# MrTornado24/FENeRF

Measured on NVIDIA H100. Metric: rendered faces/sec at 128px x 24 samples/ray, higher is better.
Workload: dtype f16 operands / f32 accumulate (wgmma) + f32 refinement

## Files before the change

### fenerf_b200/csrc/mapping.cu

```cuda
#include "common.cuh"

namespace fn {

namespace {

constexpr int kMaxB = 32;
constexpr unsigned kFull = 0xffffffffu;

struct HiddenArgs {
    const float* w[4];
    const float* b[4];
    const float* z;
    float* h_out;
    int B, z_dim;
};

constexpr int kChunkB = 8;

__global__ void __launch_bounds__(256) mapping_hidden_kernel(HiddenArgs a) {
    extern __shared__ __align__(16) float xs[];
    const int warp = threadIdx.x >> 5, lane = threadIdx.x & 31;
    const int B = a.B;
    float* x0 = xs;
    float* x1 = xs + (size_t)B * 512;
    for (int i = threadIdx.x; i < B * a.z_dim; i += blockDim.x) x0[(i / a.z_dim) * 512 + (i % a.z_dim)] = a.z[i];
    __syncthreads();
    int K = a.z_dim;
    for (int layer = 0; layer < 4; ++layer) {
        const float* W = a.w[layer];
        const float* bias = a.b[layer];
        const float* xin = (layer & 1) ? x1 : x0;
        float* xout = (layer & 1) ? x0 : x1;
#pragma unroll 1
        for (int og = 0; og < 4; ++og) {
        float4 wreg[8][4];
#pragma unroll
        for (int o = 0; o < 8; ++o)
#pragma unroll
            for (int it = 0; it < 4; ++it) {
                const int k = lane * 4 + it * 128;
                wreg[o][it] = k < K ? __ldg(reinterpret_cast<const float4*>(W + (size_t)(warp * 32 + og * 8 + o) * K + k)) : make_float4(0.f, 0.f, 0.f, 0.f);
            }
#pragma unroll
        for (int o = 0; o < 8; ++o) {
            const int f = warp * 32 + og * 8 + o;
            for (int b0 = 0; b0 < B; b0 += kChunkB) {
                float acc[kChunkB];
#pragma unroll
                for (int b = 0; b < kChunkB; ++b) acc[b] = 0.f;
#pragma unroll
                for (int it = 0; it < 4; ++it) {
                    const int k = lane * 4 + it * 128;
                    if (k < K) {
                        const float4 wv = wreg[o][it];
#pragma unroll
                        for (int b = 0; b < kChunkB; ++b)
                            if (b0 + b < B) {
                                const float4 xv = *reinterpret_cast<const float4*>(xin + (b0 + b) * 512 + k);
                                acc[b] = fmaf(wv.x, xv.x, fmaf(wv.y, xv.y, fmaf(wv.z, xv.z, fmaf(wv.w, xv.w, acc[b]))));
                            }
                    }
                }
#pragma unroll
                for (int b = 0; b < kChunkB; ++b)
                    if (b0 + b < B) {
                        float v = acc[b];
#pragma unroll
                        for (int off = 16; off > 0; off >>= 1) v += __shfl_xor_sync(kFull, v, off);
                        v += bias[f];
                        v = v > 0.f ? v : 0.2f * v;
                        if (lane == 0) {
                            if (layer == 3) a.h_out[(b0 + b) * 256 + f] = v;
                            else xout[(b0 + b) * 512 + f] = v;
                        }
                    }
            }
        }
        }
        __syncthreads();
        K = 256;
    }
}

struct OutArgs {
    const float* w;
    const float* b;
    const float* h;
    const float* avg_f;
    const float* avg_p;
    float* film;
    int B, n_layers, layer0, n_film_total;
    float psi;
};

__global__ void __launch_bounds__(256) mapping_out_kernel(OutArgs a) {
    extern __shared__ __align__(16) float hs[];
    const int B = a.B;
    for (int i = threadIdx.x; i < B * 256; i += blockDim.x) hs[i] = a.h[i];
    __syncthreads();
    const int warp = threadIdx.x >> 5, lane = threadIdx.x & 31;
    const int half = a.n_layers * 256, n_out = 2 * half;
    for (int r = blockIdx.x * 8 + warp; r < n_out; r += gridDim.x * 8) {
        const float4 w0 = *reinterpret_cast<const float4*>(a.w + (size_t)r * 256 + lane * 8);
        const float4 w1 = *reinterpret_cast<const float4*>(a.w + (size_t)r * 256 + lane * 8 + 4);
        const float bias = a.b[r];
        const bool is_freq = r < half;
        const int j = is_freq ? r : r - half, l = j >> 8, f = j & 255;
        for (int b = 0; b < B; ++b) {
            const float4 x0 = *reinterpret_cast<const float4*>(hs + b * 256 + lane * 8);
            const float4 x1 = *reinterpret_cast<const float4*>(hs + b * 256 + lane * 8 + 4);
            float v = fmaf(w0.x, x0.x, fmaf(w0.y, x0.y, fmaf(w0.z, x0.z, w0.w * x0.w)));
            v = fmaf(w1.x, x1.x, fmaf(w1.y, x1.y, fmaf(w1.z, x1.z, fmaf(w1.w, x1.w, v))));
#pragma unroll
            for (int off = 16; off > 0; off >>= 1) v += __shfl_xor_sync(kFull, v, off);
            if (lane == 0) {
                v += bias;
                if (a.avg_f) {
                    const float avg = is_freq ? a.avg_f[j] : a.avg_p[j];
                    v = __fadd_rn(avg, __fmul_rn(a.psi, __fsub_rn(v, avg)));
                }
                if (is_freq) v = __fadd_rn(__fmul_rn(v, 15.f), 30.f);
                a.film[(((size_t)b * a.n_film_total + a.layer0 + l) * 2 + (is_freq ? 0 : 1)) * 256 + f] = v;
            }
        }
    }
}

}

int mapping_film(const float* const* w, const float* const* b, const float* z, int B, int z_dim, int n_layers, int layer0,
                 int n_film_total, const float* avg_f, const float* avg_p, float psi, float* h_scratch, float* film,
                 cudaStream_t st) {
    FN_REQUIRE(z_dim >= 4 && z_dim <= 512 && z_dim % 4 == 0, "z_dim %d unsupported (multiple of 4, <= 512)", z_dim);
    for (int b0 = 0; b0 < B; b0 += kMaxB) {
        const int nb = (B - b0) < kMaxB ? (B - b0) : kMaxB;
        HiddenArgs ha;
        for (int i = 0; i < 4; ++i) { ha.w[i] = w[i]; ha.b[i] = b[i]; }
        ha.z = z + (size_t)b0 * z_dim; ha.h_out = h_scratch; ha.B = nb; ha.z_dim = z_dim;
        const size_t smem_h = (size_t)2 * nb * 512 * sizeof(float);
        static std::atomic<int> set_h[kMaxDevices];
        if (smem_h > 48 * 1024) FN_CUDA_OK(ensure_dynamic_smem(mapping_hidden_kernel, set_h, (int)smem_h));
        mapping_hidden_kernel<<<1, 256, smem_h, st>>>(ha);
        FN_LAUNCH_OK("mapping_hidden_kernel");
        OutArgs oa;
        oa.w = w[4]; oa.b = b[4]; oa.h = h_scratch; oa.avg_f = avg_f; oa.avg_p = avg_p;
        oa.film = film + (size_t)b0 * n_film_total * 512; oa.B = nb; oa.n_layers = n_layers; oa.layer0 = layer0;
        oa.n_film_total = n_film_total; oa.psi = psi;
        const int rows = n_layers * 512;
        int blocks = (rows + 7) / 8;
        if (blocks > num_sms() * 2) blocks = num_sms() * 2;
        mapping_out_kernel<<<blocks, 256, (size_t)nb * 256 * sizeof(float), st>>>(oa);
        FN_LAUNCH_OK("mapping_out_kernel");
    }
    return 0;
}

}
```

### fenerf_b200/csrc/siren_fast.cu

```cuda
#include "siren_fast.cuh"

namespace fn {

int siren_fast_label_launch(const void* args, int blocks, cudaStream_t st);
int siren_fast_hd_launch(const void* args, int blocks, bool label_film, cudaStream_t st);
int siren_fast_grid_launch(const void* args, int blocks, cudaStream_t st);
int siren_fast_bridge_launch(const void* args, int blocks, cudaStream_t st);
int siren_fast_debug_launch(const void* args, int blocks, bool label_film, bool feature_head, int variant, cudaStream_t st);

namespace {

std::atomic<int> g_variant{0};
unsigned long long* g_trace = nullptr;
int g_trace_ctas = 0;

bool build_loads(const FnLayout& L, FastArgs& A, bool sigma_only) {
    A.n_loads = 0;
    auto push = [&](size_t src, uint32_t bytes) {
        if (A.n_loads < MAX_LOADS) A.loads[A.n_loads] = Load{(uint32_t)src, bytes};
        ++A.n_loads;
    };
    push(L.first_img, 2 * CHUNK);
    if (L.grid_trunk) push(L.first_img_lo, 2 * CHUNK);
    for (int l = 0; l < L.n_hidden; ++l) {
        if (l == L.trunk_hidden) {
            push(L.head_img, 4 * HEAD_CHUNK);
            if (sigma_only) return A.n_loads <= MAX_LOADS;
        }
        if (L.bridge && l == L.color0) {
            push(L.color0_ximg, 2 * CHUNK);
            continue;
        }
        push(L.hid_img[l], 2 * CHUNK);
        push(L.hid_img[l] + 2 * CHUNK, 2 * CHUNK);
        if (l == L.label_layer) push(L.label.img, (uint32_t)FN_HEAD_IMG_BYTES(L.label.img_rows));
        if (l == L.color0) push(L.color0_ximg, 2 * CHUNK);
        push(L.hid_img[l] + 4 * CHUNK, 2 * CHUNK);
        push(L.hid_img[l] + 6 * CHUNK, 2 * CHUNK);
    }
    push(L.rgb.img, (uint32_t)FN_HEAD_IMG_BYTES(L.rgb.img_rows));
    return A.n_loads <= MAX_LOADS;
}

}

int siren_fast_debug_variant(int variant, unsigned long long* trace, int trace_ctas) {
    FN_REQUIRE(variant >= 0 && variant <= 3, "unknown point-network variant %d", variant);
    FN_REQUIRE(variant < 2 || (trace && trace_ctas >= 1), "a timeline variant needs its trace buffer");
    g_trace = trace;
    g_trace_ctas = trace_ctas;
    g_variant.store(variant);
    return 0;
}

int siren_points_fast(const FnLayout& L, const unsigned char* packed, const float* points, const float* dirs, const float* film,
                      int batch, long long ppb, int dir_group, int lock_dirs, float* out, int sigma_only, cudaStream_t st,
                      float* sigma_out) {
    static_assert(sizeof(FastArgs) <= 4000, "kernel parameter block too large");
    static_assert(SMEM_TOTAL <= 232448, "one CTA per SM: 227 KB of shared memory");
    static_assert(FN_HEAD_IMG_BYTES(FN_FEAT) == SLOT_BYTES, "a feature-head image is one ring slot");
    const bool trunk_only = L.feature_head && sigma_only;
    const bool feature_head = L.feature_head && !trunk_only, label_film = L.label_film && !trunk_only;
    FN_REQUIRE(L.trunk_hidden >= 1 && L.n_hidden - L.color0 >= 1, "field needs >= 2 trunk and >= 1 colour layers");
    FN_REQUIRE(L.sigma_row < 32, "the fast path packs labels and sigma into one 32-column head (label_dim <= 31)");
    FN_REQUIRE(L.rgb.img < 0xFFFFFFFFull && L.label.img < 0xFFFFFFFFull && L.first_img_lo < 0xFFFFFFFFull,
               "packed weight images beyond 4 GB");
    FN_REQUIRE(((uintptr_t)film & 15) == 0, "the FiLM table must be 16-byte aligned");
    FastArgs a;
    memset(&a, 0, sizeof(a));
    FN_REQUIRE(build_loads(L, a, sigma_only != 0), "field too deep for the weight stream");
    a.sigma_only = sigma_only ? 1 : 0;
    a.L = L; a.packed = packed; a.points = points; a.dirs = dirs; a.film = film; a.out = out; a.sigma_out = sigma_out;
    a.ppb = ppb; a.tiles_per_batch = (ppb + TILE - 1) / TILE; a.n_tiles = a.tiles_per_batch * batch;
    a.dir_group = dir_group < 1 ? 1 : dir_group; a.lock_dirs = lock_dirs;
    if (a.n_tiles <= 0) return 0;
    FN_REQUIRE(ppb % a.dir_group == 0, "points_per_batch %lld not a multiple of dir_group %d", ppb, a.dir_group);
    const long long n_pairs = (a.n_tiles + 1) / 2;
    static std::atomic<int> attr_set[kMaxDevices];
    const int blocks = (int)(n_pairs < (long long)num_sms() ? n_pairs : (long long)num_sms());
    if (const int variant = g_variant.load()) {
        FN_REQUIRE(!L.grid_trunk && !L.bridge,
                   "the debug point-network variants do not cover fields with the grid in the trunk or a bridge");
        a.trace = g_trace;
        a.trace_ctas = g_trace_ctas;
        return siren_fast_debug_launch(&a, blocks, label_film, feature_head, variant, st);
    }
    if (L.grid_trunk) return siren_fast_grid_launch(&a, blocks, st);
    if (L.bridge) return siren_fast_bridge_launch(&a, blocks, st);
    if (feature_head) return siren_fast_hd_launch(&a, blocks, label_film, st);
    if (label_film) return siren_fast_label_launch(&a, blocks, st);
    FN_CUDA_OK(ensure_dynamic_smem(siren_fast_kernel<false>, attr_set, (int)SMEM_TOTAL));
    siren_fast_kernel<false><<<blocks, NTHREADS, SMEM_TOTAL, st>>>(a);
    FN_LAUNCH_OK("siren_fast_kernel");
    return 0;
}

}
```

### fenerf_b200/csrc/siren_fast.cuh

```cuda
#pragma once
#include "common.cuh"
#include "siren_common.cuh"
#include "sm90.cuh"

namespace fn {

namespace {

using namespace sm90;

constexpr int TILE = 64;
constexpr int NTHREADS = 384;
constexpr int PROD_WARP = 8;
constexpr int RING = 6;
constexpr uint32_t SLOT_BYTES = 32768;
constexpr int XSTRIDE = 72;
constexpr uint32_t SMEM_X = RING * SLOT_BYTES;
constexpr int FRING = 2;
constexpr uint32_t FILM_BYTES = 2 * FN_H * 4;
constexpr uint32_t SMEM_FILM = SMEM_X + 2 * TILE * XSTRIDE * 2;
constexpr uint32_t SMEM_BAR = SMEM_FILM + 2 * FRING * FILM_BYTES;
constexpr uint32_t SMEM_TOTAL = SMEM_BAR + 16 * RING + 16 + 16 * 2 * FRING;
constexpr uint32_t SMEM_XLO = SMEM_TOTAL;
constexpr int XLO_STRIDE = 32;
constexpr uint32_t SMEM_TOTAL_GRID = SMEM_XLO + 2 * TILE * XLO_STRIDE * 2;
constexpr int MAX_LOADS = 72;
constexpr uint32_t CHUNK = 16384;
constexpr uint32_t HEAD_CHUNK = 32 * 128;
constexpr uint32_t RGB_CHUNK = 8 * 128;
constexpr uint32_t FEAT_CHUNK = FN_FEAT * 128;
#ifndef FENERF_SOFT_SIN_EVERY
#define FENERF_SOFT_SIN_EVERY 0
#endif
constexpr int kSoftSinEvery = FENERF_SOFT_SIN_EVERY;
constexpr int kSoftSinSplit = 4;
constexpr int TRACE_CAP = 1024;
constexpr int TRACE_WARPS = 11;
enum TraceEvent {
    TR_PAIR = 1, TR_TURN_WAIT, TR_TURN_DONE, TR_ACQ_WAIT, TR_ACQ_DONE, TR_COMMIT, TR_MMA_DONE, TR_EPI_DONE,
    TR_FILM_WAIT, TR_FILM_DONE, TR_EMPTY_WAIT, TR_EMPTY_DONE,
};
enum TraceGroup { TG_FIRST = 0, TG_HIDDEN, TG_COLOR0, TG_TRUNK_HEAD, TG_LABEL_LAYER, TG_LABEL_HEAD, TG_OUT_HEAD };

__device__ __forceinline__ float soft_sinf(float a) {
    const float k = fmaf(a, 0.159154943f, 12582912.f);
    const float n = k - 12582912.f;
    float r = fmaf(-n, 6.28318548f, a);
    r = fmaf(-n, -1.74845553e-7f, r);
    const float r2 = r * r;
    float p = -2.041572245e-08f;
    p = fmaf(p, r2, 2.701100129e-06f);
    p = fmaf(p, r2, -1.980991656e-04f);
    p = fmaf(p, r2, 8.332454599e-03f);
    p = fmaf(p, r2, -1.666656137e-01f);
    p = fmaf(p, r2, 9.999996424e-01f);
    return r * p;
}

struct Load {
    uint32_t src;
    uint32_t bytes;
};

struct FastArgs {
    Load loads[MAX_LOADS];
    int n_loads;
    FnLayout L;
    const unsigned char* packed;
    const float* points;
    const float* dirs;
    const float* film;
    float* out;
    float* sigma_out;
    long long ppb, tiles_per_batch, n_tiles;
    int dir_group, lock_dirs;
    int sigma_only;
    unsigned long long* trace;
    int trace_ctas;
};

__device__ __forceinline__ void wg_bar(int wg) { asm volatile("bar.sync %0, 128;" ::"r"(1 + wg) : "memory"); }

template <bool kLabelFilm, bool kFeatureHead = false, int kSoftSin = kSoftSinEvery, bool kTrace = false,
          bool kGridTrunk = false, bool kBridge = false>
__global__ void __launch_bounds__(NTHREADS, 1) siren_fast_kernel(const __grid_constant__ FastArgs a) {
    extern __shared__ __align__(1024) unsigned char smem[];
    const uint32_t sbase = smem_u32(smem);
    const int warp = threadIdx.x >> 5, lane = threadIdx.x & 31;
    const uint32_t bar_full = sbase + SMEM_BAR, bar_empty = bar_full + 8 * RING, bar_turn = bar_empty + 8 * RING;
    const uint32_t bar_ffull = bar_turn + 16, bar_fempty = bar_ffull + 8 * 2 * FRING;
    unsigned long long* tbuf = nullptr;
    uint32_t tn = 0;
    if constexpr (kTrace)
        if (lane == 0 && (int)blockIdx.x < a.trace_ctas) tbuf = a.trace + ((size_t)blockIdx.x * TRACE_WARPS + warp) * TRACE_CAP;
    auto trace = [&](int kind, int group = 0) {
        if constexpr (kTrace)
            if (tbuf && tn < TRACE_CAP)
                tbuf[tn++] = ((unsigned long long)kind << 56) | ((unsigned long long)group << 48) |
                             ((unsigned long long)clock64() & ((1ull << 48) - 1));
    };
    if (threadIdx.x == 0) {
        for (int i = 0; i < RING; ++i) {
            mbar_init(bar_full + 8 * i, 1);
            mbar_init(bar_empty + 8 * i, 8);
        }
        for (int g = 0; g < 2; ++g) mbar_init(bar_turn + 8 * g, 4);
        for (int e = 0; e < 2 * FRING; ++e) {
            mbar_init(bar_ffull + 8 * e, 32);
            mbar_init(bar_fempty + 8 * e, 4);
        }
        fence_barrier_init();
    }
    __syncthreads();
    const long long n_pairs = (a.n_tiles + 1) / 2;

    if (warp >= PROD_WARP) {
        asm volatile("setmaxnreg.dec.sync.aligned.u32 40;\n" ::: "memory");
        if (warp == PROD_WARP && lane == 0) {
            uint32_t it = 0;
            for (long long pair = blockIdx.x; pair < n_pairs; pair += gridDim.x)
                for (int i = 0; i < a.n_loads; ++i, ++it) {
                    const uint32_t slot = it % RING;
                    trace(TR_EMPTY_WAIT);
                    mbar_wait(bar_empty + 8 * slot, ((it / RING) & 1u) ^ 1u);
                    trace(TR_EMPTY_DONE);
                    mbar_arrive_expect_tx(bar_full + 8 * slot, a.loads[i].bytes);
                    bulk_g2s(sbase + slot * SLOT_BYTES, a.packed + a.loads[i].src, a.loads[i].bytes, bar_full + 8 * slot);
                }
        } else if (warp == PROD_WARP + 1 || warp == PROD_WARP + 2) {
            const int g = warp - PROD_WARP - 1;
            const int n_film = 1 + (a.sigma_only ? a.L.trunk_hidden : a.L.n_hidden);
            uint32_t it = 0;
            for (long long pair = blockIdx.x; pair < n_pairs; pair += gridDim.x) {
                const long long tile = pair * 2 + g;
                const long long b = tile < a.n_tiles ? tile / a.tiles_per_batch : 0;
                const float* film_b = a.film + (size_t)b * a.L.n_film * 2 * FN_H;
                for (int i = 0; i < n_film; ++i, ++it) {
                    const uint32_t e = g * FRING + it % FRING;
                    const float2* row = reinterpret_cast<const float2*>(film_b + (size_t)i * 2 * FN_H);
                    const float2* bias = reinterpret_cast<const float2*>(a.packed + (i == 0 ? a.L.first_b : a.L.hid_b[i - 1]));
                    float4* dst = reinterpret_cast<float4*>(smem + SMEM_FILM + e * FILM_BYTES);
                    trace(TR_EMPTY_WAIT);
                    mbar_wait(bar_fempty + 8 * e, ((it / FRING) & 1u) ^ 1u);
                    trace(TR_EMPTY_DONE);
#pragma unroll 1
                    for (int k = 0; k < FN_H / 64; ++k) {
                        const int cp = lane + 32 * k;
                        const float2 f = __ldg(row + cp), p = __ldg(row + FN_H / 2 + cp), bb = __ldg(bias + cp);
                        dst[cp] = make_float4(f.x, f.y, fmaf(f.x, bb.x, p.x), fmaf(f.y, bb.y, p.y));
                    }
                    mbar_arrive(bar_ffull + 8 * e);
                }
            }
        }
        return;
    }

    asm volatile("setmaxnreg.inc.sync.aligned.u32 232;\n" ::: "memory");
    const int wg = warp >> 2, q = lane & 3;
    const int tid = threadIdx.x & 127;
    const int r0 = (warp & 3) * 16 + (lane >> 2);
    const FnLayout& L = a.L;
    const int C = L.out_dim;
    const float* sigma_w = reinterpret_cast<const float*>(a.packed + L.sigma_w);
    const float* label_w = reinterpret_cast<const float*>(a.packed + L.label_w);
    const int trunk_labels = (kLabelFilm || kFeatureHead) ? 0 : L.trunk_labels;
    const int sigma_row = kFeatureHead ? FN_FEAT_SIGMA_ROW : L.sigma_row;
    const int rgb_rows = kFeatureHead ? FN_FEAT : L.rgb.w_rows;
    const int label_rows = kFeatureHead ? FN_FEAT : L.label.w_rows;
    __half* xs = reinterpret_cast<__half*>(smem + SMEM_X) + wg * TILE * XSTRIDE;
    uint32_t it = 0;
    auto acquire = [&](uint32_t& slot) -> uint32_t {
        slot = it % RING;
        trace(TR_ACQ_WAIT);
        mbar_wait(bar_full + 8 * slot, (it / RING) & 1u);
        trace(TR_ACQ_DONE);
        ++it;
        return sbase + slot * SLOT_BYTES;
    };
    auto release = [&](uint32_t slot) {
        __syncwarp();
        if (lane == 0) mbar_arrive(bar_empty + 8 * slot);
    };
    uint32_t turns = 0;
    uint32_t fit = 0;
    auto film_acquire = [&]() -> const float4* {
        const uint32_t e = wg * FRING + fit % FRING;
        trace(TR_FILM_WAIT);
        mbar_wait(bar_ffull + 8 * e, (fit / FRING) & 1u);
        trace(TR_FILM_DONE);
        return reinterpret_cast<const float4*>(smem + SMEM_FILM + e * FILM_BYTES);
    };
    auto film_release = [&]() {
        const uint32_t e = wg * FRING + fit % FRING;
        ++fit;
        __syncwarp();
        if (lane == 0) mbar_arrive(bar_fempty + 8 * e);
    };
    auto turn_begin = [&]() {
        trace(TR_TURN_WAIT);
        mbar_wait(bar_turn + 8 * wg, (turns & 1u) ^ (wg == 0 ? 1u : 0u));
        trace(TR_TURN_DONE);
    };
    auto turn_end = [&](int group) {
        trace(TR_COMMIT, group);
        ++turns;
        __syncwarp();
        if (lane == 0) mbar_arrive(bar_turn + 8 * (wg ^ 1));
    };
    auto xfrag = [&](int s, uint32_t (&f)[4]) {
        const __half* p = xs + r0 * XSTRIDE + 16 * s + 2 * q;
        f[0] = *reinterpret_cast<const uint32_t*>(p);
        f[1] = *reinterpret_cast<const uint32_t*>(p + 8 * XSTRIDE);
        f[2] = *reinterpret_cast<const uint32_t*>(p + 8);
        f[3] = *reinterpret_cast<const uint32_t*>(p + 8 * XSTRIDE + 8);
    };

    for (long long pair = blockIdx.x; pair < n_pairs; pair += gridDim.x) {
        const long long tile = pair * 2 + wg;
        const bool tile_ok = tile < a.n_tiles;
        const long long b = tile_ok ? tile / a.tiles_per_batch : 0;
        const long long p0 = tile_ok ? (tile % a.tiles_per_batch) * TILE : a.ppb;
        trace(TR_PAIR);

        wg_bar(wg);
        if (tid < TILE) {
            float pos[3] = {0.f, 0.f, 0.f}, dir[3] = {0.f, 0.f, 0.f};
            const long long pp = p0 + tid;
            const bool valid = pp < a.ppb;
            if (valid) {
                const long long ff = b * a.ppb + pp;
#pragma unroll
                for (int i = 0; i < 3; ++i) pos[i] = __fmul_rn(a.points[ff * 3 + i], L.input_scale);
                if (a.lock_dirs) dir[2] = -1.f;
                else {
                    const long long di = b * (a.ppb / a.dir_group) + pp / a.dir_group;
#pragma unroll
                    for (int i = 0; i < 3; ++i) dir[i] = a.dirs[di * 3 + i];
                }
            }
            __align__(16) __half slots[64];
#pragma unroll
            for (int i = 0; i < 64; ++i) slots[i] = __float2half_rn(0.f);
#pragma unroll
            for (int i = 0; i < 3; ++i) {
                __half hi, lo;
                split_f16(pos[i], hi, lo);
                slots[FN_SLOT_POS + i] = hi; slots[FN_SLOT_POS + 3 + i] = lo; slots[FN_SLOT_POS + 6 + i] = hi;
                split_f16(dir[i], hi, lo);
                slots[FN_SLOT_DIR + i] = hi; slots[FN_SLOT_DIR + 3 + i] = lo; slots[FN_SLOT_DIR + 6 + i] = hi;
            }
            if constexpr (kGridTrunk) {
                __align__(16) __half lo[32];
#pragma unroll
                for (int i = 0; i < 32; ++i) lo[i] = __float2half_rn(0.f);
                if (valid) {
                    float feat[32];
                    grid_features32(reinterpret_cast<const float*>(a.packed + L.grid), L.grid_res, pos[0], pos[1], pos[2], feat);
#pragma unroll
                    for (int i = 0; i < 32; ++i) split_f16(feat[i], slots[FN_SLOT_FEAT + i], lo[i]);
                }
                __half* xlo = reinterpret_cast<__half*>(smem + SMEM_XLO) + (wg * TILE + tid) * XLO_STRIDE;
#pragma unroll
                for (int i = 0; i < 4; ++i) reinterpret_cast<uint4*>(xlo)[i] = reinterpret_cast<const uint4*>(lo)[i];
            } else if (L.grid_channels > 0 && valid && !a.sigma_only) {
                float feat[32];
                grid_features32_h(reinterpret_cast<const __half*>(a.packed + L.grid16), L.grid_res, pos[0], pos[1], pos[2], feat);
#pragma unroll
                for (int i = 0; i < 32; ++i) slots[FN_SLOT_FEAT + i] = __float2half_rn(feat[i]);
            }
#pragma unroll
            for (int i = 0; i < 8; ++i)
                reinterpret_cast<uint4*>(xs + tid * XSTRIDE)[i] = reinterpret_cast<const uint4*>(slots)[i];
        }
        wg_bar(wg);

        uint32_t act[16][4];
        uint32_t nxt[8][4];
        float d[64];
        auto film_epi = [&](const float4* fs, int h, uint32_t (&dst)[8][4]) {
#pragma unroll
            for (int j = 0; j < 16; ++j) {
                const float4 e = fs[64 * h + 4 * j + q];
                const bool soft = kSoftSin > 0 && j % (kSoftSin > 0 ? kSoftSin : 1) == kSoftSin - 1;
                auto sn = [soft](float x) { return soft ? soft_sinf(x) : __sinf(x); };
                dst[j >> 1][(j & 1) * 2] = pack_half2(sn(fmaf(e.x, d[4 * j], e.z)), sn(fmaf(e.y, d[4 * j + 1], e.w)));
                dst[j >> 1][(j & 1) * 2 + 1] = pack_half2(sn(fmaf(e.x, d[4 * j + 2], e.z)), sn(fmaf(e.y, d[4 * j + 3], e.w)));
            }
            trace(TR_EPI_DONE);
        };
        auto act_hi = [&]() -> uint32_t (&)[8][4] { return *reinterpret_cast<uint32_t (*)[8][4]>(&act[8]); };

        {
            uint32_t xf[4], slot, slot_lo = 0, w_lo = 0;
            uint32_t xg[2][4], xl[2][4];
            const float4* fs = nullptr;
            xfrag(0, xf);
            if constexpr (kGridTrunk) {
                const __half* xlo = reinterpret_cast<const __half*>(smem + SMEM_XLO) + wg * TILE * XLO_STRIDE;
#pragma unroll
                for (int s = 0; s < 2; ++s) {
                    xfrag(2 + s, xg[s]);
                    const __half* p = xlo + r0 * XLO_STRIDE + 16 * s + 2 * q;
                    xl[s][0] = *reinterpret_cast<const uint32_t*>(p);
                    xl[s][1] = *reinterpret_cast<const uint32_t*>(p + 8 * XLO_STRIDE);
                    xl[s][2] = *reinterpret_cast<const uint32_t*>(p + 8);
                    xl[s][3] = *reinterpret_cast<const uint32_t*>(p + 8 * XLO_STRIDE + 8);
                }
            }
            const uint32_t w = acquire(slot);
            if constexpr (kGridTrunk) w_lo = acquire(slot_lo);
#pragma unroll
            for (int h = 0; h < 2; ++h) {
                turn_begin();
                wg_fence();
                mma_rs_n128(d, xf, desc_kmajor(w + h * CHUNK), 0u);
                if constexpr (kGridTrunk)
#pragma unroll
                    for (int s = 0; s < 2; ++s) {
                        mma_rs_n128(d, xg[s], desc_kmajor(w + h * CHUNK + 32 * (2 + s)), 1u);
                        mma_rs_n128(d, xl[s], desc_kmajor(w + h * CHUNK + 32 * (2 + s)), 1u);
                        mma_rs_n128(d, xg[s], desc_kmajor(w_lo + h * CHUNK + 32 * (2 + s)), 1u);
                    }
                wg_commit();
                turn_end(TG_FIRST);
                wg_wait<0>();
                trace(TR_MMA_DONE);
                fence_regs(d);
                fence_regs(xf);
                if constexpr (kGridTrunk) { fence_regs(xg); fence_regs(xl); }
                if (h == 0) fs = film_acquire();
                if (h == 0) film_epi(fs, 0, nxt);
                else film_epi(fs, 1, act_hi());
            }
            release(slot);
            if constexpr (kGridTrunk) release(slot_lo);
            film_release();
#pragma unroll
            for (int s = 0; s < 8; ++s)
#pragma unroll
                for (int i = 0; i < 4; ++i) act[s][i] = nxt[s][i];
        }

        bool stop = false;
        for (int l = 0; l < L.n_hidden && !stop; ++l) {
            if (l == L.trunk_hidden) {
                float dh[16];
                uint32_t slot;
                const uint32_t w = acquire(slot);
                turn_begin();
                wg_fence();
#pragma unroll
                for (int c = 0; c < 4; ++c)
#pragma unroll
                    for (int k = 0; k < 4; ++k) mma_rs_n32(dh, act[4 * c + k], desc_kmajor(w + c * HEAD_CHUNK + 32 * k), (c | k) ? 1u : 0u);
                wg_commit();
                turn_end(TG_TRUNK_HEAD);
                wg_wait<0>();
                trace(TR_MMA_DONE);
                fence_regs(dh);
                fence_regs(act);
                release(slot);
                const float* lb = label_w + FENERF_MAX_LABEL * FN_H;
#pragma unroll
                for (int rr = 0; rr < 2; ++rr) {
                    const long long pnt = p0 + r0 + 8 * rr;
                    if (pnt >= a.ppb) continue;
                    const long long flat = b * a.ppb + pnt;
#pragma unroll
                    for (int i = 0; i < 4; ++i)
#pragma unroll
                        for (int e = 0; e < 2; ++e) {
                            const int o = 8 * i + 2 * q + e;
                            const float v = dh[4 * i + 2 * rr + e];
                            if (o < trunk_labels) {
                                if (!a.sigma_only) a.out[flat * C + o] = fmaf(v, __ldg(lb + FENERF_MAX_LABEL), __ldg(lb + o));
                            } else if (o == sigma_row && !(kBridge && L.bridge_res)) {
                                const float sig = v + __ldg(sigma_w + FN_H);
                                a.out[flat * C + (C - 1)] = sig;
                                if (a.sigma_out) a.sigma_out[flat] = sig;
                            }
                        }
                }
                if constexpr (kBridge) {
                    const float* bw = reinterpret_cast<const float*>(a.packed + L.bridge_w);
#pragma unroll
                    for (int rr = 0; rr < 2; ++rr) {
                        const float o0 = dh[2 * rr], o1 = dh[2 * rr + 1];
                        const float p2 = __shfl_xor_sync(0xffffffffu, o0, 1), p3 = __shfl_xor_sync(0xffffffffu, o1, 1);
                        if (q != 0) continue;
                        const long long pnt = p0 + r0 + 8 * rr;
                        float v[3] = {o1 + __ldg(bw + 3 * FN_H), p2 + __ldg(bw + 3 * FN_H + 1), p3 + __ldg(bw + 3 * FN_H + 2)};
                        if (L.bridge_res) {
                            if (pnt < a.ppb) {
                                const long long flat = b * a.ppb + pnt;
#pragma unroll
                                for (int j = 0; j < 3; ++j) v[j] += __fmul_rn(a.points[flat * 3 + j], L.input_scale);
                                float sig = __ldg(bw + 3 * FN_H + 6);
#pragma unroll
                                for (int j = 0; j < 3; ++j) sig = fmaf(__ldg(bw + 3 * FN_H + 3 + j), v[j], sig);
                                a.out[flat * C + (C - 1)] = sig;
                                if (a.sigma_out) a.sigma_out[flat] = sig;
                            }
                        }
                        if (!a.sigma_only) {
                            __half* row = xs + (r0 + 8 * rr) * XSTRIDE + FN_SLOT_FEAT;
#pragma unroll
                            for (int j = 0; j < 3; ++j) {
                                __half hi, lo;
                                split_f16(v[j], hi, lo);
                                row[j] = hi; row[3 + j] = lo; row[6 + j] = hi;
                            }
                        }
                    }
                    if (!a.sigma_only) wg_bar(wg);
                }
                if (a.sigma_only) { stop = true; break; }
                if constexpr (kLabelFilm) {
                    constexpr int kLabN = kFeatureHead ? FN_FEAT : 32;
                    constexpr uint32_t kLabChunk = kFeatureHead ? FEAT_CHUNK : HEAD_CHUNK;
                    float dl[kLabN / 2];
                    uint32_t slot_h = 0, w_h = 0;
                    const float4* fs = nullptr;
#pragma unroll
                    for (int h = 0; h < 2; ++h) {
                        uint32_t sl[2];
                        turn_begin();
                        wg_fence();
#pragma unroll
                        for (int sb = 0; sb < 2; ++sb) {
                            const uint32_t w = acquire(sl[sb]);
#pragma unroll
                            for (int c = 0; c < 2; ++c)
#pragma unroll
                                for (int k = 0; k < 4; ++k)
                                    mma_rs_n128(d, act[8 * sb + 4 * c + k], desc_kmajor(w + c * CHUNK + 32 * k), (sb | c | k) ? 1u : 0u);
                        }
                        wg_commit();
                        turn_end(TG_LABEL_LAYER);
                        wg_wait<0>();
                        trace(TR_MMA_DONE);
                        fence_regs(d);
                        fence_regs(act);
                        release(sl[0]);
                        release(sl[1]);
                        if (h == 0) fs = film_acquire();
                        film_epi(fs, h, nxt);
                        if (h == 0) w_h = acquire(slot_h);
                        turn_begin();
                        wg_fence();
#pragma unroll
                        for (int s = 0; s < 8; ++s) {
                            const int g = 8 * h + s;
                            const uint64_t desc = desc_kmajor(w_h + (g >> 2) * kLabChunk + 32 * (g & 3));
                            if constexpr (kFeatureHead) mma_rs_n64(dl, nxt[s], desc, (h | s) ? 1u : 0u);
                            else mma_rs_n32(dl, nxt[s], desc, (h | s) ? 1u : 0u);
                        }
                        wg_commit();
                        turn_end(TG_LABEL_HEAD);
                        wg_wait<0>();
                        trace(TR_MMA_DONE);
                        fence_regs(dl);
                        fence_regs(nxt);
                    }
                    release(slot_h);
                    film_release();
#pragma unroll
                    for (int rr = 0; rr < 2; ++rr) {
                        const long long pnt = p0 + r0 + 8 * rr;
                        if (pnt >= a.ppb) continue;
                        const long long flat = b * a.ppb + pnt;
                        const float* lbias = reinterpret_cast<const float*>(a.packed + L.label.w) + label_rows * FN_H;
#pragma unroll
                        for (int i = 0; i < kLabN / 8; ++i)
#pragma unroll
                            for (int e = 0; e < 2; ++e) {
                                const int o = 8 * i + 2 * q + e;
                                if (o < L.label.n_out) a.out[flat * C + o] = dl[4 * i + 2 * rr + e] + __ldg(lbias + o);
                            }
                    }
                    continue;
                }
            }
            const bool c0 = (l == L.color0);
            const bool narrow = kBridge && c0;
            const int nx = kBridge ? 2 : !kGridTrunk && L.grid_channels > 0 ? 3 : 1;
            uint32_t xf[3][4];
            if (c0)
#pragma unroll
                for (int s = 0; s < 3; ++s) xfrag(1 + s, xf[s]);
            uint32_t slot_x = 0, w_x = 0;
            const float4* fs = nullptr;
#pragma unroll
            for (int h = 0; h < 2; ++h) {
                uint32_t sl[2] = {0u, 0u};
                if (narrow && h == 0) w_x = acquire(slot_x);
                turn_begin();
                wg_fence();
                if (!narrow)
#pragma unroll
                    for (int sb = 0; sb < 2; ++sb) {
                        const uint32_t w = acquire(sl[sb]);
#pragma unroll
                        for (int c = 0; c < 2; ++c)
#pragma unroll
                            for (int k = 0; k < 4; ++k)
                                mma_rs_n128(d, act[8 * sb + 4 * c + k], desc_kmajor(w + c * CHUNK + 32 * k), (sb | c | k) ? 1u : 0u);
                    }
                if (c0) {
                    if (h == 0 && !narrow) w_x = acquire(slot_x);
#pragma unroll
                    for (int s = 0; s < 3; ++s)
                        if (s < nx) mma_rs_n128(d, xf[s], desc_kmajor(w_x + h * CHUNK + 32 * (1 + s)), (narrow && s == 0) ? 0u : 1u);
                }
                wg_commit();
                turn_end(c0 ? TG_COLOR0 : TG_HIDDEN);
                wg_wait<0>();
                trace(TR_MMA_DONE);
                fence_regs(d);
                fence_regs(act);
                fence_regs(xf);
                if (!narrow) {
                    release(sl[0]);
                    release(sl[1]);
                }
                if (c0 && h == 1) release(slot_x);
                if (h == 0) fs = film_acquire();
                if (h == 0) film_epi(fs, 0, nxt);
                else film_epi(fs, 1, act_hi());
            }
            film_release();
#pragma unroll
            for (int s = 0; s < 8; ++s)
#pragma unroll
                for (int i = 0; i < 4; ++i) act[s][i] = nxt[s][i];
        }
        if (stop) continue;

        if constexpr (kFeatureHead) {
            float dr[32];
            uint32_t slot;
            const uint32_t w = acquire(slot);
            turn_begin();
            wg_fence();
#pragma unroll
            for (int c = 0; c < 4; ++c)
#pragma unroll
                for (int k = 0; k < 4; ++k) mma_rs_n64(dr, act[4 * c + k], desc_kmajor(w + c * FEAT_CHUNK + 32 * k), (c | k) ? 1u : 0u);
            wg_commit();
            turn_end(TG_OUT_HEAD);
            wg_wait<0>();
            trace(TR_MMA_DONE);
            fence_regs(dr);
            fence_regs(act);
            release(slot);
            const float* rgb_b = reinterpret_cast<const float*>(a.packed + L.rgb.w) + rgb_rows * FN_H;
#pragma unroll
            for (int rr = 0; rr < 2; ++rr) {
                const long long pnt = p0 + r0 + 8 * rr;
                if (pnt >= a.ppb) continue;
                const long long flat = b * a.ppb + pnt;
#pragma unroll
                for (int i = 0; i < 8; ++i)
#pragma unroll
                    for (int e = 0; e < 2; ++e) {
                        const int o = 8 * i + 2 * q + e;
                        a.out[flat * C + L.label_dim + o] = dr[4 * i + 2 * rr + e] + __ldg(rgb_b + o);
                    }
            }
            continue;
        }
        {
            float dr[4];
            uint32_t slot;
            const uint32_t w = acquire(slot);
            turn_begin();
            wg_fence();
#pragma unroll
            for (int c = 0; c < 4; ++c)
#pragma unroll
                for (int k = 0; k < 4; ++k) mma_rs_n8(dr, act[4 * c + k], desc_kmajor(w + c * RGB_CHUNK + 32 * k), (c | k) ? 1u : 0u);
            wg_commit();
            turn_end(TG_OUT_HEAD);
            wg_wait<0>();
            trace(TR_MMA_DONE);
            fence_regs(dr);
            fence_regs(act);
            release(slot);
            const float* rgb_b = reinterpret_cast<const float*>(a.packed + L.rgb.w) + rgb_rows * FN_H;
#pragma unroll
            for (int rr = 0; rr < 2; ++rr) {
                const long long pnt = p0 + r0 + 8 * rr;
                if (pnt >= a.ppb) continue;
                const long long flat = b * a.ppb + pnt;
#pragma unroll
                for (int e = 0; e < 2; ++e) {
                    const int o = 2 * q + e;
                    if (o < 3) {
                        const float x = dr[2 * rr + e] + __ldg(rgb_b + o);
                        a.out[flat * C + L.label_dim + o] = __fdividef(1.f, 1.f + __expf(-x));
                    }
                }
            }
        }
    }
}

}

}
```

### fenerf_b200/csrc/siren_fast_debug.cu

```cuda
#include "siren_fast.cuh"

namespace fn {

namespace {

template <bool kLabelFilm, bool kFeatureHead, int kSoftSin, bool kTrace>
int launch(const FastArgs& a, int blocks, cudaStream_t st) {
    static std::atomic<int> attr_set[kMaxDevices];
    FN_CUDA_OK(ensure_dynamic_smem(siren_fast_kernel<kLabelFilm, kFeatureHead, kSoftSin, kTrace>, attr_set, (int)SMEM_TOTAL));
    siren_fast_kernel<kLabelFilm, kFeatureHead, kSoftSin, kTrace><<<blocks, NTHREADS, SMEM_TOTAL, st>>>(a);
    FN_LAUNCH_OK("siren_fast_kernel<debug>");
    return 0;
}

__global__ void soft_sine_kernel(const float* a, float* out, long long n) {
    const long long i = (long long)blockIdx.x * blockDim.x + threadIdx.x;
    if (i < n) out[i] = soft_sinf(a[i]);
}

}

int siren_fast_debug_launch(const void* args, int blocks, bool label_film, bool feature_head, int variant, cudaStream_t st) {
    const FastArgs& a = *static_cast<const FastArgs*>(args);
    if (variant == 1) {
        if (feature_head) return label_film ? launch<true, true, kSoftSinSplit, false>(a, blocks, st) : launch<false, true, kSoftSinSplit, false>(a, blocks, st);
        return label_film ? launch<true, false, kSoftSinSplit, false>(a, blocks, st) : launch<false, false, kSoftSinSplit, false>(a, blocks, st);
    }
    FN_REQUIRE(!label_film && !feature_head, "the point-network timeline covers plain fields only");
    if (variant == 2) return launch<false, false, kSoftSinEvery, true>(a, blocks, st);
    return launch<false, false, kSoftSinSplit, true>(a, blocks, st);
}

int soft_sine_eval(const float* a, float* out, long long n, cudaStream_t st) {
    if (n <= 0) return 0;
    soft_sine_kernel<<<(unsigned)((n + 255) / 256), 256, 0, st>>>(a, out, n);
    FN_LAUNCH_OK("soft_sine_kernel");
    return 0;
}

}
```

Baseline: 601.8.

## Split mapping MLP into per-layer multi-block launches and add stream/MMA ablation variants

The four hidden layers of the mapping network previously ran in a single-block kernel that looped over all layers in shared memory. They now run as one launch per layer across 32 blocks, each warp computing a single output feature, with intermediates passed through global memory (film buffer and h_scratch as scratch). This spreads the serial mapping work over many SMs, at the cost of extra launches and global round-trips, and it reuses the film buffer as temporary storage. Separately, the debug path gains ablation variants that disable either the weight stream or the MMAs, which are off by default.

Result: faster. 616.9 (median of 6 runs) (+2.5%).

```diff
diff --git a/fenerf_b200/csrc/mapping.cu b/fenerf_b200/csrc/mapping.cu
--- a/fenerf_b200/csrc/mapping.cu
+++ b/fenerf_b200/csrc/mapping.cu
@@ -7,78 +7,55 @@
 constexpr int kMaxB = 32;
 constexpr unsigned kFull = 0xffffffffu;
 
-struct HiddenArgs {
-    const float* w[4];
-    const float* b[4];
-    const float* z;
-    float* h_out;
-    int B, z_dim;
+struct LayerArgs {
+    const float* w;
+    const float* b;
+    const float* x;
+    float* y;
+    long long x_stride, y_stride;
+    int B, K;
 };
 
 constexpr int kChunkB = 8;
 
-__global__ void __launch_bounds__(256) mapping_hidden_kernel(HiddenArgs a) {
-    extern __shared__ __align__(16) float xs[];
+__global__ void __launch_bounds__(256) mapping_layer_kernel(LayerArgs a) {
     const int warp = threadIdx.x >> 5, lane = threadIdx.x & 31;
-    const int B = a.B;
-    float* x0 = xs;
-    float* x1 = xs + (size_t)B * 512;
-    for (int i = threadIdx.x; i < B * a.z_dim; i += blockDim.x) x0[(i / a.z_dim) * 512 + (i % a.z_dim)] = a.z[i];
-    __syncthreads();
-    int K = a.z_dim;
-    for (int layer = 0; layer < 4; ++layer) {
-        const float* W = a.w[layer];
-        const float* bias = a.b[layer];
-        const float* xin = (layer & 1) ? x1 : x0;
-        float* xout = (layer & 1) ? x0 : x1;
-#pragma unroll 1
-        for (int og = 0; og < 4; ++og) {
-        float4 wreg[8][4];
+    const int f = blockIdx.x * 8 + warp;
+    float4 wreg[4];
 #pragma unroll
-        for (int o = 0; o < 8; ++o)
+    for (int it = 0; it < 4; ++it) {
+        const int k = lane * 4 + it * 128;
+        wreg[it] = k < a.K ? __ldg(reinterpret_cast<const float4*>(a.w + (size_t)f * a.K + k)) : make_float4(0.f, 0.f, 0.f, 0.f);
+    }
+    const float bias = __ldg(a.b + f);
+    for (int b0 = 0; b0 < a.B; b0 += kChunkB) {
+        float acc[kChunkB];
 #pragma unroll
-            for (int it = 0; it < 4; ++it) {
-                const int k = lane * 4 + it * 128;
-                wreg[o][it] = k < K ? __ldg(reinterpret_cast<const float4*>(W + (size_t)(warp * 32 + og * 8 + o) * K + k)) : make_float4(0.f, 0.f, 0.f, 0.f);
-            }
+        for (int b = 0; b < kChunkB; ++b) acc[b] = 0.f;
 #pragma unroll
-        for (int o = 0; o < 8; ++o) {
-            const int f = warp * 32 + og * 8 + o;
-            for (int b0 = 0; b0 < B; b0 += kChunkB) {
-                float acc[kChunkB];
-#pragma unroll
-                for (int b = 0; b < kChunkB; ++b) acc[b] = 0.f;
-#pragma unroll
-                for (int it = 0; it < 4; ++it) {
-                    const int k = lane * 4 + it * 128;
-                    if (k < K) {
-                        const float4 wv = wreg[o][it];
-#pragma unroll
-                        for (int b = 0; b < kChunkB; ++b)
-                            if (b0 + b < B) {
-                                const float4 xv = *reinterpret_cast<const float4*>(xin + (b0 + b) * 512 + k);
-                                acc[b] = fmaf(wv.x, xv.x, fmaf(wv.y, xv.y, fmaf(wv.z, xv.z, fmaf(wv.w, xv.w, acc[b]))));
-                            }
-                    }
-                }
+        for (int it = 0; it < 4; ++it) {
+            const int k = lane * 4 + it * 128;
+            if (k < a.K) {
+                const float4 wv = wreg[it];
 #pragma unroll
                 for (int b = 0; b < kChunkB; ++b)
-                    if (b0 + b < B) {
-                        float v = acc[b];
-#pragma unroll
-                        for (int off = 16; off > 0; off >>= 1) v += __shfl_xor_sync(kFull, v, off);
-                        v += bias[f];
-                        v = v > 0.f ? v : 0.2f * v;
-                        if (lane == 0) {
-                            if (layer == 3) a.h_out[(b0 + b) * 256 + f] = v;
-                            else xout[(b0 + b) * 512 + f] = v;
-                        }
+                    if (b0 + b < a.B) {
+                        const float* xp = a.x + (b0 + b) * a.x_stride + k;
+                        const float4 xv = make_float4(__ldg(xp), __ldg(xp + 1), __ldg(xp + 2), __ldg(xp + 3));
+                        acc[b] = fmaf(wv.x, xv.x, fmaf(wv.y, xv.y, fmaf(wv.z, xv.z, fmaf(wv.w, xv.w, acc[b]))));
                     }
             }
         }
-        }
-        __syncthreads();
-        K = 256;
+#pragma unroll
+        for (int b = 0; b < kChunkB; ++b)
+            if (b0 + b < a.B) {
+                float v = acc[b];
+#pragma unroll
+                for (int off = 16; off > 0; off >>= 1) v += __shfl_xor_sync(kFull, v, off);
+                v += bias;
+                v = v > 0.f ? v : 0.2f * v;
+                if (lane == 0) a.y[(b0 + b) * a.y_stride + f] = v;
+            }
     }
 }
 
@@ -134,14 +111,19 @@
     FN_REQUIRE(z_dim >= 4 && z_dim <= 512 && z_dim % 4 == 0, "z_dim %d unsupported (multiple of 4, <= 512)", z_dim);
     for (int b0 = 0; b0 < B; b0 += kMaxB) {
         const int nb = (B - b0) < kMaxB ? (B - b0) : kMaxB;
-        HiddenArgs ha;
-        for (int i = 0; i < 4; ++i) { ha.w[i] = w[i]; ha.b[i] = b[i]; }
-        ha.z = z + (size_t)b0 * z_dim; ha.h_out = h_scratch; ha.B = nb; ha.z_dim = z_dim;
-        const size_t smem_h = (size_t)2 * nb * 512 * sizeof(float);
-        static std::atomic<int> set_h[kMaxDevices];
-        if (smem_h > 48 * 1024) FN_CUDA_OK(ensure_dynamic_smem(mapping_hidden_kernel, set_h, (int)smem_h));
-        mapping_hidden_kernel<<<1, 256, smem_h, st>>>(ha);
-        FN_LAUNCH_OK("mapping_hidden_kernel");
+        float* film_rows = film + (size_t)b0 * n_film_total * 512 + (size_t)layer0 * 512;
+        const long long film_stride = (long long)n_film_total * 512;
+        LayerArgs la;
+        la.B = nb;
+        for (int layer = 0; layer < 4; ++layer) {
+            la.w = w[layer]; la.b = b[layer];
+            if (layer == 0) { la.x = z + (size_t)b0 * z_dim; la.x_stride = z_dim; la.K = z_dim; }
+            else { la.x = la.y; la.x_stride = la.y_stride; la.K = 256; }
+            if (layer & 1) { la.y = h_scratch; la.y_stride = 256; }
+            else { la.y = film_rows; la.y_stride = film_stride; }
+            mapping_layer_kernel<<<256 / 8, 256, 0, st>>>(la);
+            FN_LAUNCH_OK("mapping_layer_kernel");
+        }
         OutArgs oa;
         oa.w = w[4]; oa.b = b[4]; oa.h = h_scratch; oa.avg_f = avg_f; oa.avg_p = avg_p;
         oa.film = film + (size_t)b0 * n_film_total * 512; oa.B = nb; oa.n_layers = n_layers; oa.layer0 = layer0;
diff --git a/fenerf_b200/csrc/siren_fast.cu b/fenerf_b200/csrc/siren_fast.cu
--- a/fenerf_b200/csrc/siren_fast.cu
+++ b/fenerf_b200/csrc/siren_fast.cu
@@ -45,8 +45,8 @@
 }
 
 int siren_fast_debug_variant(int variant, unsigned long long* trace, int trace_ctas) {
-    FN_REQUIRE(variant >= 0 && variant <= 3, "unknown point-network variant %d", variant);
-    FN_REQUIRE(variant < 2 || (trace && trace_ctas >= 1), "a timeline variant needs its trace buffer");
+    FN_REQUIRE(variant >= 0 && variant <= 5, "unknown point-network variant %d", variant);
+    FN_REQUIRE((variant != 2 && variant != 3) || (trace && trace_ctas >= 1), "a timeline variant needs its trace buffer");
     g_trace = trace;
     g_trace_ctas = trace_ctas;
     g_variant.store(variant);
diff --git a/fenerf_b200/csrc/siren_fast.cuh b/fenerf_b200/csrc/siren_fast.cuh
--- a/fenerf_b200/csrc/siren_fast.cuh
+++ b/fenerf_b200/csrc/siren_fast.cuh
@@ -41,6 +41,7 @@
     TR_FILM_WAIT, TR_FILM_DONE, TR_EMPTY_WAIT, TR_EMPTY_DONE,
 };
 enum TraceGroup { TG_FIRST = 0, TG_HIDDEN, TG_COLOR0, TG_TRUNK_HEAD, TG_LABEL_LAYER, TG_LABEL_HEAD, TG_OUT_HEAD };
+enum StreamAblation { AB_NONE = 0, AB_STREAM_ONLY, AB_NO_STREAM };
 
 __device__ __forceinline__ float soft_sinf(float a) {
     const float k = fmaf(a, 0.159154943f, 12582912.f);
@@ -82,8 +83,9 @@
 __device__ __forceinline__ void wg_bar(int wg) { asm volatile("bar.sync %0, 128;" ::"r"(1 + wg) : "memory"); }
 
 template <bool kLabelFilm, bool kFeatureHead = false, int kSoftSin = kSoftSinEvery, bool kTrace = false,
-          bool kGridTrunk = false, bool kBridge = false>
+          bool kGridTrunk = false, bool kBridge = false, int kAblate = AB_NONE>
 __global__ void __launch_bounds__(NTHREADS, 1) siren_fast_kernel(const __grid_constant__ FastArgs a) {
+    constexpr bool kMma = kAblate != AB_STREAM_ONLY, kStream = kAblate != AB_NO_STREAM;
     extern __shared__ __align__(1024) unsigned char smem[];
     const uint32_t sbase = smem_u32(smem);
     const int warp = threadIdx.x >> 5, lane = threadIdx.x & 31;
@@ -116,7 +118,7 @@
 
     if (warp >= PROD_WARP) {
         asm volatile("setmaxnreg.dec.sync.aligned.u32 40;\n" ::: "memory");
-        if (warp == PROD_WARP && lane == 0) {
+        if (warp == PROD_WARP && lane == 0 && kStream) {
             uint32_t it = 0;
             for (long long pair = blockIdx.x; pair < n_pairs; pair += gridDim.x)
                 for (int i = 0; i < a.n_loads; ++i, ++it) {
@@ -173,14 +175,14 @@
     auto acquire = [&](uint32_t& slot) -> uint32_t {
         slot = it % RING;
         trace(TR_ACQ_WAIT);
-        mbar_wait(bar_full + 8 * slot, (it / RING) & 1u);
+        if constexpr (kStream) mbar_wait(bar_full + 8 * slot, (it / RING) & 1u);
         trace(TR_ACQ_DONE);
         ++it;
         return sbase + slot * SLOT_BYTES;
     };
     auto release = [&](uint32_t slot) {
         __syncwarp();
-        if (lane == 0) mbar_arrive(bar_empty + 8 * slot);
+        if (lane == 0 && kStream) mbar_arrive(bar_empty + 8 * slot);
     };
     uint32_t turns = 0;
     uint32_t fit = 0;
@@ -280,7 +282,7 @@
         float d[64];
         auto film_epi = [&](const float4* fs, int h, uint32_t (&dst)[8][4]) {
 #pragma unroll
-            for (int j = 0; j < 16; ++j) {
+            for (int j = 0; j < (kMma ? 16 : 0); ++j) {
                 const float4 e = fs[64 * h + 4 * j + q];
                 const bool soft = kSoftSin > 0 && j % (kSoftSin > 0 ? kSoftSin : 1) == kSoftSin - 1;
                 auto sn = [soft](float x) { return soft ? soft_sinf(x) : __sinf(x); };
@@ -314,8 +316,8 @@
             for (int h = 0; h < 2; ++h) {
                 turn_begin();
                 wg_fence();
-                mma_rs_n128(d, xf, desc_kmajor(w + h * CHUNK), 0u);
-                if constexpr (kGridTrunk)
+                if constexpr (kMma) mma_rs_n128(d, xf, desc_kmajor(w + h * CHUNK), 0u);
+                if constexpr (kGridTrunk && kMma)
 #pragma unroll
                     for (int s = 0; s < 2; ++s) {
                         mma_rs_n128(d, xg[s], desc_kmajor(w + h * CHUNK + 32 * (2 + s)), 1u);
@@ -353,7 +355,8 @@
 #pragma unroll
                 for (int c = 0; c < 4; ++c)
 #pragma unroll
-                    for (int k = 0; k < 4; ++k) mma_rs_n32(dh, act[4 * c + k], desc_kmajor(w + c * HEAD_CHUNK + 32 * k), (c | k) ? 1u : 0u);
+                    for (int k = 0; k < 4; ++k)
+                        if constexpr (kMma) mma_rs_n32(dh, act[4 * c + k], desc_kmajor(w + c * HEAD_CHUNK + 32 * k), (c | k) ? 1u : 0u);
                 wg_commit();
                 turn_end(TG_TRUNK_HEAD);
                 wg_wait<0>();
@@ -434,7 +437,8 @@
                             for (int c = 0; c < 2; ++c)
 #pragma unroll
                                 for (int k = 0; k < 4; ++k)
-                                    mma_rs_n128(d, act[8 * sb + 4 * c + k], desc_kmajor(w + c * CHUNK + 32 * k), (sb | c | k) ? 1u : 0u);
+                                    if constexpr (kMma)
+                                        mma_rs_n128(d, act[8 * sb + 4 * c + k], desc_kmajor(w + c * CHUNK + 32 * k), (sb | c | k) ? 1u : 0u);
                         }
                         wg_commit();
                         turn_end(TG_LABEL_LAYER);
@@ -453,7 +457,8 @@
                         for (int s = 0; s < 8; ++s) {
                             const int g = 8 * h + s;
                             const uint64_t desc = desc_kmajor(w_h + (g >> 2) * kLabChunk + 32 * (g & 3));
-                            if constexpr (kFeatureHead) mma_rs_n64(dl, nxt[s], desc, (h | s) ? 1u : 0u);
+                            if constexpr (!kMma) (void)desc;
+                            else if constexpr (kFeatureHead) mma_rs_n64(dl, nxt[s], desc, (h | s) ? 1u : 0u);
                             else mma_rs_n32(dl, nxt[s], desc, (h | s) ? 1u : 0u);
                         }
                         wg_commit();
@@ -505,13 +510,14 @@
                         for (int c = 0; c < 2; ++c)
 #pragma unroll
                             for (int k = 0; k < 4; ++k)
-                                mma_rs_n128(d, act[8 * sb + 4 * c + k], desc_kmajor(w + c * CHUNK + 32 * k), (sb | c | k) ? 1u : 0u);
+                                if constexpr (kMma)
+                                    mma_rs_n128(d, act[8 * sb + 4 * c + k], desc_kmajor(w + c * CHUNK + 32 * k), (sb | c | k) ? 1u : 0u);
                     }
                 if (c0) {
                     if (h == 0 && !narrow) w_x = acquire(slot_x);
 #pragma unroll
                     for (int s = 0; s < 3; ++s)
-                        if (s < nx) mma_rs_n128(d, xf[s], desc_kmajor(w_x + h * CHUNK + 32 * (1 + s)), (narrow && s == 0) ? 0u : 1u);
+                        if (kMma && s < nx) mma_rs_n128(d, xf[s], desc_kmajor(w_x + h * CHUNK + 32 * (1 + s)), (narrow && s == 0) ? 0u : 1u);
                 }
                 wg_commit();
                 turn_end(c0 ? TG_COLOR0 : TG_HIDDEN);
@@ -546,7 +552,8 @@
 #pragma unroll
             for (int c = 0; c < 4; ++c)
 #pragma unroll
-                for (int k = 0; k < 4; ++k) mma_rs_n64(dr, act[4 * c + k], desc_kmajor(w + c * FEAT_CHUNK + 32 * k), (c | k) ? 1u : 0u);
+                for (int k = 0; k < 4; ++k)
+                    if constexpr (kMma) mma_rs_n64(dr, act[4 * c + k], desc_kmajor(w + c * FEAT_CHUNK + 32 * k), (c | k) ? 1u : 0u);
             wg_commit();
             turn_end(TG_OUT_HEAD);
             wg_wait<0>();
@@ -579,7 +586,8 @@
 #pragma unroll
             for (int c = 0; c < 4; ++c)
 #pragma unroll
-                for (int k = 0; k < 4; ++k) mma_rs_n8(dr, act[4 * c + k], desc_kmajor(w + c * RGB_CHUNK + 32 * k), (c | k) ? 1u : 0u);
+                for (int k = 0; k < 4; ++k)
+                    if constexpr (kMma) mma_rs_n8(dr, act[4 * c + k], desc_kmajor(w + c * RGB_CHUNK + 32 * k), (c | k) ? 1u : 0u);
             wg_commit();
             turn_end(TG_OUT_HEAD);
             wg_wait<0>();
diff --git a/fenerf_b200/csrc/siren_fast_debug.cu b/fenerf_b200/csrc/siren_fast_debug.cu
--- a/fenerf_b200/csrc/siren_fast_debug.cu
+++ b/fenerf_b200/csrc/siren_fast_debug.cu
@@ -4,13 +4,23 @@
 
 namespace {
 
-template <bool kLabelFilm, bool kFeatureHead, int kSoftSin, bool kTrace>
+template <bool kLabelFilm, bool kFeatureHead, int kSoftSin, bool kTrace, int kAblate = AB_NONE>
 int launch(const FastArgs& a, int blocks, cudaStream_t st) {
+    constexpr auto kernel = siren_fast_kernel<kLabelFilm, kFeatureHead, kSoftSin, kTrace, false, false, kAblate>;
     static std::atomic<int> attr_set[kMaxDevices];
-    FN_CUDA_OK(ensure_dynamic_smem(siren_fast_kernel<kLabelFilm, kFeatureHead, kSoftSin, kTrace>, attr_set, (int)SMEM_TOTAL));
-    siren_fast_kernel<kLabelFilm, kFeatureHead, kSoftSin, kTrace><<<blocks, NTHREADS, SMEM_TOTAL, st>>>(a);
+    FN_CUDA_OK(ensure_dynamic_smem(kernel, attr_set, (int)SMEM_TOTAL));
+    kernel<<<blocks, NTHREADS, SMEM_TOTAL, st>>>(a);
     FN_LAUNCH_OK("siren_fast_kernel<debug>");
     return 0;
+}
+
+template <int kSoftSin, int kAblate>
+int launch_any(const FastArgs& a, int blocks, bool label_film, bool feature_head, cudaStream_t st) {
+    if (feature_head)
+        return label_film ? launch<true, true, kSoftSin, false, kAblate>(a, blocks, st)
+                          : launch<false, true, kSoftSin, false, kAblate>(a, blocks, st);
+    return label_film ? launch<true, false, kSoftSin, false, kAblate>(a, blocks, st)
+                      : launch<false, false, kSoftSin, false, kAblate>(a, blocks, st);
 }
 
 __global__ void soft_sine_kernel(const float* a, float* out, long long n) {
@@ -22,10 +32,9 @@
 
 int siren_fast_debug_launch(const void* args, int blocks, bool label_film, bool feature_head, int variant, cudaStream_t st) {
     const FastArgs& a = *static_cast<const FastArgs*>(args);
-    if (variant == 1) {
-        if (feature_head) return label_film ? launch<true, true, kSoftSinSplit, false>(a, blocks, st) : launch<false, true, kSoftSinSplit, false>(a, blocks, st);
-        return label_film ? launch<true, false, kSoftSinSplit, false>(a, blocks, st) : launch<false, false, kSoftSinSplit, false>(a, blocks, st);
-    }
+    if (variant == 1) return launch_any<kSoftSinSplit, AB_NONE>(a, blocks, label_film, feature_head, st);
+    if (variant == 4) return launch_any<kSoftSinEvery, AB_STREAM_ONLY>(a, blocks, label_film, feature_head, st);
+    if (variant == 5) return launch_any<kSoftSinEvery, AB_NO_STREAM>(a, blocks, label_film, feature_head, st);
     FN_REQUIRE(!label_film && !feature_head, "the point-network timeline covers plain fields only");
     if (variant == 2) return launch<false, false, kSoftSinEvery, true>(a, blocks, st);
     return launch<false, false, kSoftSinSplit, true>(a, blocks, st);
```
